# microhh/rte-rrtmgp-cpp

Measured on AMD Instinct MI355X. Metric: columns/sec (LW+SW full solve, 140 lay x 256 gpt), higher is better.
Workload: dtype f64; 1 GPU; C4 synthetic 16384 columns/GPU (16384 in total) x 140 layers x 256 g-points, LW+SW clear-sky, RCEMIP profile, synthetic k-distribution (real shapes); columns_per_gpu=16384, columns_total=16384, nlay=140, ngpt=256, flux_mode=broadband (do_broadband solvers, g-point sums on chip), columns_sorted=False, parallelism=columns sharded x1, all-gather of broadband fluxes

## Files before the change

### include/rrx_hip.h

```cpp
#ifndef RRX_HIP_H
#define RRX_HIP_H

#ifdef __cplusplus
extern "C" {
#endif

typedef signed char RrxBool;

const char* rrx_last_error(void);
int rrx_device_count(int* n);
int rrx_set_device(int dev);
int rrx_malloc(void** ptr, unsigned long long bytes);
int rrx_free(void* ptr);
int rrx_malloc_async(void** ptr, unsigned long long bytes, void* stream);
int rrx_free_async(void* ptr, void* stream);
int rrx_free_async_ordered(void* ptr, void* alloc_stream, void* release_stream);
int rrx_memcpy_h2d_stream(void* dst, const void* src, unsigned long long bytes, void* stream);
int rrx_memcpy_d2h_stream(void* dst, const void* src, unsigned long long bytes, void* stream);
int rrx_memcpy_h2d(void* dst, const void* src, unsigned long long bytes);
int rrx_memcpy_d2h(void* dst, const void* src, unsigned long long bytes);
int rrx_memcpy_d2d(void* dst, const void* src, unsigned long long bytes, void* stream);
int rrx_memset(void* dst, int value, unsigned long long bytes, void* stream);
int rrx_synchronize(void* stream);
int rrx_stream_create(void** stream);
int rrx_stream_destroy(void* stream);
int rrx_release_workspace(void* stream);
int rrx_identity_columns(int ncol, int npad, int* perm, void* stream);
unsigned long long rrx_workspace_bytes(void* stream);
int rrx_subset_nd(void* out, const void* in, int elem_bytes, int ndim, const int* sub_dims, const long long* strides,
                  const int* starts, const int* spread, void* stream);
int rrx_set_lw_variant(int v);
int rrx_set_sw_variant(int v);
int rrx_set_broadband_min_groups(int n);
int rrx_set_broadband_gsplit(int n);
int rrx_set_gas_window(int on);
int rrx_gas_window_stats(long long* handed_back, long long* workgroups, int reset);

#define RRX_DECLARE(F, SFX) \
 \
 \
int rrx_apply_BC_factor##SFX(int ncol, int nlay, int ngpt, RrxBool top_at_1, const F* inc_flux_dir, const F* mu0, F* gpt_flux_dir, void* stream); \
int rrx_apply_BC_0##SFX(int ncol, int nlay, int ngpt, RrxBool top_at_1, F* gpt_flux_dn, void* stream); \
int rrx_apply_BC_gpt##SFX(int ncol, int nlay, int ngpt, RrxBool top_at_1, const F* inc_flux_dif, F* gpt_flux_dn, void* stream); \
 \
int rrx_lw_secants_array##SFX(int ncol, int ngpt, int n_gauss_quad, int max_gauss_pts, const F* gauss_Ds, F* secants, void* stream); \
 \
int rrx_lw_solver_noscat##SFX( \
        int ncol, int nlay, int ngpt, RrxBool top_at_1, int nmus, \
        const F* secants, const F* weights, \
        const F* tau, const F* lay_source, const F* lev_source, \
        const F* sfc_emis, const F* sfc_src, const F* inc_flux, \
// ... 306 lines not shown
```

### rte-rrtmgp-cpp_amd/csrc/rrx_gas_optics.hip

```cpp
#include <type_traits>
#include <cstdio>
#include <cstdlib>
#include "rrx_common.h"
#include "rrx_hip.h"

namespace
{
#ifndef RRX_GW_NT
#define RRX_GW_NT 1
#endif
#ifndef RRX_GW_ABL
#define RRX_GW_ABL 0
#endif
template<typename F> __device__ __forceinline__ void stream_store_sbase(const char* sbase, const unsigned voff, const F v)
{
    static_assert(sizeof(F) == 4 || sizeof(F) == 8, "dword or dwordx2");
    if (RRX_GW_ABL == 7) { if (v == F(-12345.678)) *reinterpret_cast<F*>(const_cast<char*>(sbase) + voff) = v; return; }
#if RRX_GW_NT
    if constexpr (sizeof(F) == 4) asm volatile("global_store_dword %0, %1, %2 nt" :: "v"(voff), "v"(v), "s"(sbase) : "memory");
    else asm volatile("global_store_dwordx2 %0, %1, %2 nt" :: "v"(voff), "v"(v), "s"(sbase) : "memory");
#else
    if constexpr (sizeof(F) == 4) asm volatile("global_store_dword %0, %1, %2" :: "v"(voff), "v"(v), "s"(sbase) : "memory");
    else asm volatile("global_store_dwordx2 %0, %1, %2" :: "v"(voff), "v"(v), "s"(sbase) : "memory");
#endif
// ... 1220 lines not shown
template<typename F> struct PlanckArgs
{
    const F* pfracin; const F* tlev; const F* tsfc; int sfc_lay; int nPlanckTemp; const int* gpoint_bands;
    F totplnk_delta; const F* totplnk; F* pfrac; F* blay; F* blev; F* sfc_src; F* sfc_src_jac;
};

struct GasWindowTables
{
    int ngpt, nmax, ncmax;
    static constexpr int LIT = 1 + NXW;
    __host__ __device__ int off_cinfo() const { return 2*ngpt; }
    __host__ __device__ int off_lists() const { return off_cinfo() + ncmax + 3; }
    __host__ __device__ int off_mmeta() const { return off_lists() + 2*ncmax*LIT; }
    __host__ __device__ int off_cuni()  const { return off_mmeta() + 2*MM*nmax; }
    __host__ __device__ int off_order() const { return off_cuni() + 2*ncmax; }
    __host__ __device__ int ints()      const { return (off_order() + 2*ncmax + 3) & ~3; }
};
inline int gas_window_ncmax(const int ngpt, const int nband) { return (ngpt + GCH - 1) / GCH + std::max(nband, 0); }

constexpr int GW_TBL_HEADER = 8;
constexpr int GW_TBL_MAGIC = 0x52525834;
__global__ void __launch_bounds__(256)
gas_window_tables_kernel(
        const int ngpt, const int nminorlower, const int nminorupper, const int ncmax, const int nlist,
        const int* __restrict__ gpoint_flavor,
        const int* __restrict__ minor_limits_gpt_lower, const int* __restrict__ minor_limits_gpt_upper,
        const Bool* __restrict__ minor_scales_with_density_lower, const Bool* __restrict__ minor_scales_with_density_upper,
        const Bool* __restrict__ scale_by_complement_lower, const Bool* __restrict__ scale_by_complement_upper,
        const int* __restrict__ idx_minor_lower, const int* __restrict__ idx_minor_upper,
        const int* __restrict__ idx_minor_scaling_lower, const int* __restrict__ idx_minor_scaling_upper,
        const int* __restrict__ kminor_start_lower, const int* __restrict__ kminor_start_upper,
        int* __restrict__ tbl)
{
    extern __shared__ int lds_int[];
    const int nmax = max(nminorlower, nminorupper);
    const GasWindowTables T{ngpt, nmax, ncmax};
    constexpr int LIT = GasWindowTables::LIT;
    int* gflav = lds_int;
    int* cinfo = lds_int + T.off_cinfo();
    int* lists = lds_int + T.off_lists();
    int* mmeta = lds_int + T.off_mmeta();
    int* cuni = lds_int + T.off_cuni();
    int* order = lds_int + T.off_order();
    int* cut = lds_int + T.ints();
    const int tid = threadIdx.x;
    const int ntab = T.ints();
    for (int w = tid; w < ntab + ngpt + 4 + 2*((ngpt + 63)/64); w += 256) lds_int[w] = 0;
    __syncthreads();
    {
        for (int w = tid; w < 2*ngpt; w += 256) gflav[(w & 1)*ngpt + (w >> 1)] = gpoint_flavor[w] - 1;
        for (int w = tid; w < nminorlower; w += 256)
        {
            int* m = mmeta + MM*w;
            m[0] = idx_minor_lower[w]; m[1] = minor_scales_with_density_lower[w] ? 1 : 0;
            m[2] = idx_minor_scaling_lower[w]; m[3] = scale_by_complement_lower[w] ? 1 : 0;
            m[4] = minor_limits_gpt_lower[2*w]; m[5] = minor_limits_gpt_lower[2*w+1]; m[6] = kminor_start_lower[w];
        }
        for (int w = tid; w < nminorupper; w += 256)
        {
            int* m = mmeta + MM*(nmax + w);
            m[0] = idx_minor_upper[w]; m[1] = minor_scales_with_density_upper[w] ? 1 : 0;
            m[2] = idx_minor_scaling_upper[w]; m[3] = scale_by_complement_upper[w] ? 1 : 0;
            m[4] = minor_limits_gpt_upper[2*w]; m[5] = minor_limits_gpt_upper[2*w+1]; m[6] = kminor_start_upper[w];
        }
    }
    __syncthreads();
    {
        int* head = tbl + ntab;
        int differs = (head[0] != GW_TBL_MAGIC || head[1] != ngpt || head[2] != nminorlower || head[3] != nminorupper
                       || head[4] != ncmax || head[5] != nlist) ? 1 : 0;
        for (int w = tid; w < 2*ngpt && !differs; w += 256) differs = (tbl[w] != gflav[w]) ? 1 : 0;
        for (int w = tid; w < 2*MM*nmax && !differs; w += 256) differs = (tbl[T.off_mmeta() + w] != mmeta[w]) ? 1 : 0;
        if (!__syncthreads_or(differs)) return;
        if (tid == 0) head[0] = 0;
    }
    for (int g = tid; g < ngpt; g += 256)
        if (g > 0 && (gflav[g] != gflav[g-1] || gflav[ngpt + g] != gflav[ngpt + g-1])) cut[g] = 1;
    for (int w = tid; w < 2*nmax; w += 256)
    {
        const int r = w / nmax, i = w % nmax;
        if (i < (r == 0 ? nminorlower : nminorupper))
        {
            const int* m = mmeta + MM*w;
            const int lo = m[4]-1, hi = m[5];
            if (lo > 0 && lo < ngpt) cut[lo] = 1;
            if (hi > 0 && hi < ngpt) cut[hi] = 1;
        }
// ... 74 lines not shown
            for (int d=c; d<nchunk; ++d) if (gflav[tid*ngpt + cinfo[2 + d]] == fl) ord[k++] = d;
        }
    }

    __syncthreads();
#ifdef RRX_GW_DEBUG_TABLES
    if (tid == 0)
    {
        printf("tables: ngpt %d ncmax %d chunks %d regular %d\n", ngpt, ncmax, cinfo[0], cinfo[1]);
        for (int c=0; c<nchunk; ++c)
            printf("  chunk %d [%d,%d) lower: n %d usable %d fl %d | upper: n %d usable %d fl %d\n", c, cinfo[2+c], cinfo[3+c],
                   lists[c*LIT], cuni[c], gflav[cinfo[2+c]], lists[(ncmax + c)*LIT], cuni[ncmax + c], gflav[ngpt + cinfo[2+c]]);
    }
#endif
    for (int w = tid; w < ntab; w += 256) tbl[w] = lds_int[w];
    __threadfence();
    __syncthreads();
    if (tid == 0)
    {
        int* head = tbl + ntab;
        head[1] = ngpt; head[2] = nminorlower; head[3] = nminorupper; head[4] = ncmax; head[5] = nlist;
        __threadfence();
        head[0] = GW_TBL_MAGIC;
    }
}

inline int* gas_window_tables(hipStream_t st, const int* key_ptr, const int ngpt, const int nminorlower, const int nminorupper,
                              const int ncmax, const int nlist)
{
    struct Entry { int dev; const int* key; int dims[5]; int* buf; };
    static thread_local std::vector<Entry> cache;
    int dev = 0;
    if (hipGetDevice(&dev) != hipSuccess) throw std::runtime_error("no device");
    const int dims[5] = {ngpt, nminorlower, nminorupper, ncmax, nlist};
    for (const Entry& e : cache)
        if (e.dev == dev && e.key == key_ptr && std::equal(dims, dims + 5, e.dims)) return e.buf;
    (void)st;
    if (cache.size() >= 32) { (void)hipFree(cache.front().buf); cache.erase(cache.begin()); }
    const size_t n = size_t(GasWindowTables{ngpt, std::max(nminorlower, nminorupper), ncmax}.ints()) + GW_TBL_HEADER;
    Entry e{dev, key_ptr, {dims[0], dims[1], dims[2], dims[3], dims[4]}, nullptr};
    if (hipMalloc(reinterpret_cast<void**>(&e.buf), n*sizeof(int)) != hipSuccess) throw std::runtime_error("table allocation failed");
    if (hipMemset(e.buf, 0, n*sizeof(int)) != hipSuccess) throw std::runtime_error("memset failed");
    cache.push_back(e);
    return e.buf;
}

template<typename F>
size_t gas_window_lds_bytes(const int ngpt, const int nmax, const int ncmax, const int mode, const bool pf)
{
    const size_t ints = size_t(GasWindowTables{ngpt, nmax, ncmax}.ints()) + 16 + 8*size_t(ncmax);
    const size_t pairs = size_t(GCH)*WBOX*(pf ? 2 : 1) + size_t(NCW)*GCH*MBOX + (mode == 1 ? size_t(GCH)*MBOX : 0);
    return ((ints*sizeof(int) + 15) & ~size_t(15)) + pairs*2*sizeof(F);
}

#ifndef RRX_GW_MINW
#define RRX_GW_MINW 3
#endif
template<typename F, int MODE, bool PF, bool CLD = false>
__global__ void __launch_bounds__(256, RRX_GW_MINW)
gas_window_kernel(
        const int ncol, const int nlay, const int ngpt, const int neta, const int npres, const int ntemp,
        const int nminorlower, const int nminorupper, const int idx_h2o,
        const int* __restrict__ gpoint_flavor,
        const F* __restrict__ kmajor, const F* __restrict__ kminor_lower, const F* __restrict__ kminor_upper,
        const int* __restrict__ minor_limits_gpt_lower, const int* __restrict__ minor_limits_gpt_upper,
// ... 2 lines not shown
        const int* __restrict__ idx_minor_lower, const int* __restrict__ idx_minor_upper,
        const int* __restrict__ idx_minor_scaling_lower, const int* __restrict__ idx_minor_scaling_upper,
        const int* __restrict__ kminor_start_lower, const int* __restrict__ kminor_start_upper,
        const F* __restrict__ play, const F* __restrict__ tlay, const F* __restrict__ col_gas, const F* __restrict__ col_dry,
        const F* __restrict__ krayl, const InterpArgs<F> ia,
        F* __restrict__ tau, F* __restrict__ ssa, F* __restrict__ g, const PlanckArgs<F> pa,
        int* __restrict__ todo, const int geom, const int* __restrict__ tbl, const int ncmax)
{
    #pragma clang fp contract(fast)
    typedef F Vec2 __attribute__((ext_vector_type(2)));
    typedef F Vec2u __attribute__((ext_vector_type(2), aligned(sizeof(F))));
    (void)sizeof(Vec2u);
    extern __shared__ int lds_int[];
    const int nmax = max(nminorlower, nminorupper);
    const GasWindowTables T{ngpt, nmax, ncmax};
    constexpr int LIT = GasWindowTables::LIT;
    int* gflav = lds_int;
    const int* cinfo = lds_int + T.off_cinfo();
    const int* cstart = cinfo + 2;
    int* lists = lds_int + T.off_lists();
    int* mmeta = lds_int + T.off_mmeta();
    int* cuni = lds_int + T.off_cuni();
    int* red = lds_int + T.ints();
    int* cband = red + 16;
    const size_t int_bytes = ((size_t(T.ints()) + 16 + 8*size_t(ncmax))*sizeof(int) + 15) & ~size_t(15);
    Vec2* Wmaj = reinterpret_cast<Vec2*>(reinterpret_cast<char*>(lds_int) + int_bytes);
    Vec2* Wpf  = Wmaj + GCH*WBOX;
    Vec2* Wmin = Wpf + (PF ? GCH*WBOX : 0);
    Vec2* Wray = Wmin + NCW*GCH*MBOX;

    const int tid = threadIdx.y*64 + threadIdx.x;
#if RRX_GW_TIMING
    unsigned long long gw_acc[8] = {0, 0, 0, 0, 0, 0, 0, 0}, gw_t = __builtin_readcyclecounter();
#endif
    {
        const int n4 = T.ints() / 4;
        const int4* __restrict__ src = reinterpret_cast<const int4*>(tbl);
        int4* dst = reinterpret_cast<int4*>(lds_int);
        for (int w = tid; w < n4; w += 256) dst[w] = src[w];
        if (tid < 16) red[tid] = (tid >= 6) ? 0 : ((tid & 1) ? -2147483647 : 2147483647);
    }

    const int icol_raw = geom ? (blockIdx.x*4 + threadIdx.y)*64 + threadIdx.x : blockIdx.x*64 + threadIdx.x;
    const int ilay_raw = geom ? int(blockIdx.y) : blockIdx.y*4 + threadIdx.y;
    const bool active = icol_raw < ncol && ilay_raw < nlay;
    const int icol = min(icol_raw, ncol-1), ilay = min(ilay_raw, nlay-1);
    const size_t ncl = size_t(ncol)*nlay;
    const size_t idx = icol + size_t(ilay)*ncol;
    const F pl = play[idx], tl = tlay[idx];
    const CellState<F> cs = cell_state<F>(ia, npres, ntemp, pl, tl);
    const int itr = cs.itropo;
    const int jt = cs.jt, jp = cs.jp_raw + itr;

    __syncthreads();
    atomicMin(&red[0], jt); atomicMax(&red[1], jt); atomicMin(&red[2], jp); atomicMax(&red[3], jp);
    atomicMin(&red[4], itr); atomicMax(&red[5], itr);
    if (tid < cinfo[0])
    {
        const int c0_ = cstart[tid], ge_ = cstart[tid+1];
        if constexpr (PF) { cband[8*tid] = pa.gpoint_bands[c0_] - 1; cband[8*tid+1] = pa.gpoint_bands[ge_-1] - 1; }
        if constexpr (CLD)
        {
            int b0 = 0;
            while (c0_ + 1 > ia.cld_lims[2*b0+1]) ++b0;
            cband[8*tid+2] = b0; cband[8*tid+3] = (ge_ <= ia.cld_lims[2*b0+1]) ? 1 : 0;
        }
        #pragma unroll
        for (int r=0; r<2; ++r)
        {
            const int fl_ = gflav[r*ngpt + c0_];
            cband[8*tid+4+2*r] = ia.flavor[2*fl_]; cband[8*tid+5+2*r] = ia.flavor[2*fl_+1];
        }
    }
    __syncthreads();
    const int jt_lo = red[0], jp_lo = red[2];
    const int nchunk = rfl(cinfo[0]);
    const bool whole_range = gridDim.z > 1 && rfl(cinfo[1]) == 0;
    if (whole_range && blockIdx.z > 0) return;
    const int c_per = whole_range ? nchunk : (nchunk + int(gridDim.z) - 1) / int(gridDim.z);
    const int c_lo = whole_range ? 0 : int(blockIdx.z)*c_per, c_hi = min(nchunk, c_lo + c_per);
    bool fits = (red[1] - jt_lo < NTW) && (red[3] - jp_lo + 2 <= NPW) && (red[4] == red[5]);
    {
        bool all_chunks = true;
        for (int c=c_lo; c<c_hi; ++c) all_chunks = all_chunks && (cuni[itr*ncmax + c] != 0);
        fits = fits && all_chunks;
    }
    auto hand_back = [&](const int why)
    {
        if (tid == 0)
        {
            const int k = atomicAdd(&todo[0], 1);
            todo[1 + k] = int(blockIdx.y*gridDim.x + blockIdx.x) + int(whole_range ? gridDim.z : blockIdx.z)*int(gridDim.x*gridDim.y);
            atomicAdd(&todo[why - 8], 1);
        }
    };
    if (!fits)
    {
        hand_back(!(red[1] - jt_lo < NTW) ? 0 : !(red[3] - jp_lo + 2 <= NPW) ? 1 : (red[4] != red[5]) ? 2 : 3);
        return;
    }
// ... 1 lines not shown
    const int tn = ntemp*neta;
    const size_t s_gpt = size_t(ntemp)*neta*(npres+1);
    constexpr unsigned SZ = sizeof(F);
    const F cdry0 = col_gas[idx];
    const F ch2o = col_gas[idx + size_t(idx_h2o)*ncl];
    F ray_fac = F(0.);
    if constexpr (MODE == 1) ray_fac = ch2o + col_dry[idx];
    const int ti = jt - jt_lo;
    const int pi0 = jp - jp_lo;

    const unsigned idx_b = unsigned(idx)*SZ;
    auto slab_store = [&](F* __restrict__ arr, const int ig, const F v)
    {
        stream_store(reinterpret_cast<F*>(reinterpret_cast<char*>(arr + size_t(ig)*ncl) + idx_b), v);
    };
    auto minor_scaling = [&](const int imnr) -> F
    {
        const int* m = mmeta + MM*(itr*nmax + imnr);
        const int imn = rfl(m[0]), swd = rfl(m[1]), ims = rfl(m[2]), sbc = rfl(m[3]);
        F scaling = col_gas[idx + size_t(imn)*ncl];
        const F cscal = col_gas[idx + size_t(max(ims, 0))*ncl];
        if (swd)
        {
            scaling *= F(0.01) * pl / tl;
            if (ims > 0)
            {
                const F vmr_fact = F(1.) / cdry0;
                const F dry_fact = F(1.) / (F(1.) + ch2o * vmr_fact);
                const F x = cscal * vmr_fact * dry_fact;
                scaling *= sbc ? (F(1.) - x) : x;
            }
        }
        return scaling;
    };

    [[maybe_unused]] F b_sfc = F(0.), b_sfc2 = F(0.);
    [[maybe_unused]] bool is_last = false, is_sfc = false;
    [[maybe_unused]] int cur_bnd = -1;
    [[maybe_unused]] const size_t ncv = size_t(ncol)*(nlay+1);
    [[maybe_unused]] F t_lev = F(0.);
    if constexpr (PF)
    {
        is_last = ilay == nlay-1; is_sfc = ilay == pa.sfc_lay-1;
        t_lev = pa.tlev[idx];
    }
    if constexpr (PF)
    {
        const int b_first = rfl(cband[8*c_lo]), b_last = rfl(cband[8*(c_hi-1)+1]);
        const size_t ncv_ = size_t(ncol)*(nlay+1);
        const Interp1dPos<F> p_lay = interp1d_pos(tl, ia.temp_ref_min, pa.totplnk_delta, pa.nPlanckTemp);
        const Interp1dPos<F> p_lev = interp1d_pos(t_lev, ia.temp_ref_min, pa.totplnk_delta, pa.nPlanckTemp);
        Interp1dPos<F> p_levp = p_lev;
        if (is_last) p_levp = interp1d_pos(pa.tlev[idx + ncol], ia.temp_ref_min, pa.totplnk_delta, pa.nPlanckTemp);
        #pragma unroll 4
        for (int ib=b_first; ib<=b_last; ++ib)
        {
            const F* tp = pa.totplnk + size_t(ib)*pa.nPlanckTemp;
            const F bl = interp1d_at(p_lay, tp), bv = interp1d_at(p_lev, tp);
            if (active) { pa.blay[idx + size_t(ib)*ncl] = bl; pa.blev[idx + size_t(ib)*ncv_] = bv; }
            if (is_last && active) pa.blev[idx + ncol + size_t(ib)*ncv_] = interp1d_at(p_levp, tp);
        }
    }


    int cur_flav = -1, je_lo = 1;
    [[maybe_unused]] int ne_x = NEW;
    [[maybe_unused]] int cb = 0, cb_have = -1;
    [[maybe_unused]] F c_tau = F(0.), c_ssa = F(0.), c_g = F(0.);
    F fm[8], cm[2], fn[4]; int je[2] = {1, 1};
    #pragma unroll
    for (int i=0; i<8; ++i) fm[i] = F(0.);
    cm[0] = cm[1] = F(0.); fn[0] = fn[1] = fn[2] = fn[3] = F(0.);
    const F* kmin = itr == 0 ? kminor_lower : kminor_upper;
    int red_slot = 6;

    if (RRX_GW_ABL == 1) return;
    RRX_GW_T(0)
    const int* corder = lds_int + T.off_order() + rfl(itr)*ncmax;
    auto item_meta = [&](const int* items, const int i, int& lo, int& hi, int& koff)
    {
        const int* m = mmeta + MM*(rfl(itr)*nmax + rfl(items[i]));
        lo = rfl(m[4]) - 1; hi = rfl(m[5]); koff = rfl(m[6]) - 1 - lo;
    };
    for (int kc=c_lo; kc<c_hi; ++kc)
    {
        const int c = (gridDim.z == 1 || whole_range) ? rfl(corder[kc]) : kc;
        const int c0 = rfl(cstart[c]), gend = rfl(cstart[c+1]), ng = gend - c0;
        const int fl = gflav[itr*ngpt + c0];
        if (fl != cur_flav)
        {
            cur_flav = fl;
            const int gas1 = rfl(cband[8*c+4+2*rfl(itr)]), gas2 = rfl(cband[8*c+5+2*rfl(itr)]);
            const F cg1 = col_gas[idx + size_t(gas1)*ncl], cg2 = col_gas[idx + size_t(gas2)*ncl];
            #pragma unroll
            for (int itemp=0; itemp<2; ++itemp)
            {
                F fmi[2], fma[4];
                flavor_state<F>(ia, cs, neta, itemp, gas1, gas2, cg1, cg2, cm[itemp], je[itemp], fmi, fma);
                fn[2*itemp] = fmi[0]; fn[2*itemp+1] = fmi[1];
                fm[4*itemp] = fma[0]; fm[4*itemp+1] = fma[1]; fm[4*itemp+2] = fma[2]; fm[4*itemp+3] = fma[3];
            }
            unsigned present = 0u;
            for (int j=1; j<neta; ++j)
                if (__ballot(je[0] == j || je[1] == j) != 0ull) present |= (1u << j);
            if (threadIdx.x == 0) atomicOr(reinterpret_cast<unsigned*>(&red[red_slot]), present);
            __syncthreads();
            const unsigned all_present = reinterpret_cast<unsigned*>(red)[red_slot];
            je_lo = __ffs(int(all_present)) - 1;
            const int je_hi = 31 - __clz(int(all_present));
            red_slot = (red_slot == 6) ? 8 : 6;
            if (tid == 0) red[red_slot] = 0;
            if (je_hi - je_lo + 2 > NEW) { hand_back(4); return; }
            ne_x = je_hi - je_lo + 2;
        }
        const int itr_s = rfl(itr);
        const int n_all = rfl(lists[(itr_s*ncmax + c)*LIT]);
        const int n = min(n_all, NCW);
        const int* items = lists + (itr_s*ncmax + c)*LIT + 1;

        [[maybe_unused]] auto cld_arrived = [&]()
        {
            if constexpr (CLD)
            {
                if constexpr (MODE != 2) asm volatile("" : "+v"(c_tau), "+v"(c_ssa), "+v"(c_g));
                else asm volatile("" : "+v"(c_tau));
            }
        };
        [[maybe_unused]] auto cld_load = [&](const int ib)
        {
            if constexpr (CLD)
            {
                cb_have = ib;
                const size_t b = idx + size_t(ib)*ncl;
                c_tau = ia.cld_tau[b];
                if constexpr (MODE != 2) { c_ssa = ia.cld_ssa[b]; c_g = ia.cld_g[b]; }
            }
        };
        [[maybe_unused]] bool cld_one_band = false;
        if constexpr (CLD)
        {
            const int b0 = rfl(cband[8*c+2]);
            cb = b0;
            cld_one_band = rfl(cband[8*c+3]) != 0;
            if (cld_one_band && b0 != cb_have) cld_load(b0);
        }

        RRX_GW_T(1)
        __syncthreads();
        RRX_GW_T(4)
        F sc[NCW]; int slo[NCW], shi[NCW], skoff[NCW];
        auto chunk_scalings = [&]()
        {
            #pragma unroll
            for (int i=0; i<NCW; ++i)
            {
                sc[i] = F(0.); slo[i] = 0; shi[i] = 0; skoff[i] = 0;
                if (i < n) { sc[i] = minor_scaling(rfl(items[i])); item_meta(items, i, slo[i], shi[i], skoff[i]); }
            }
        };
        if (RRX_GW_ABL != 2)
        {
            static_assert((GCH*WBOX) % 256 == 0 && GCH*MBOX <= 256 && NCW == 6, "staging phases are written for these box sizes");
            constexpr int KMAJ = GCH*WBOX/256;
            const int nmaj = ng*WBOX, nmin = ng*MBOX;
            constexpr bool DMA = RRX_GW_LDSDMA && sizeof(F) == 8;
            if constexpr (!DMA || PF) chunk_scalings();
            if constexpr (RRX_GW_SPARSE && (PF || !DMA))
            {
                auto magic = [](const int d) -> unsigned { return 0xFFFFFFFFu / unsigned(d) + 1u; };
                auto divs = [](const int x, const int d, const unsigned m) -> int { return d == 1 ? x : int(__umulhi(unsigned(x), m)); };
                const int np_x = rfl(red[3]) - jp_lo + 2, nt_x = rfl(red[1]) - jt_lo + 1;
                const int et = ne_x*nt_x, wb = np_x*et;
// ... 64 lines not shown
                const int it_ = min(jt_lo - 1 + t, ntemp-2), ie = min(max(je_lo - 1 + e, 0), neta-1), ip = min(max(jp_lo - 1 + p, 0), npres);
                const unsigned off = (unsigned(c0 + gi)*unsigned(s_gpt) + unsigned(it_ + ie*ntemp + ip*tn))*SZ;
                glds(byte_off(kmajor, off), Wmaj + q);
                if constexpr (PF) glds(byte_off(pa.pfracin, off), Wpf + q);
            }
            if (tid < GCH*MBOX)
            {
                const int gi_m = min(tid / MBOX, ng-1), r_m = tid % MBOX;
                const int it_m = min(jt_lo - 1 + r_m % NTW, ntemp-2), ie_m = min(max(je_lo - 1 + r_m / NTW, 0), neta-1);
                if constexpr (MODE == 1)
                    glds(byte_off(krayl + size_t(rfl(itr))*tn*ngpt, unsigned((c0 + gi_m)*tn + it_m + ie_m*ntemp)*SZ), Wray + tid);
                #pragma unroll
                for (int i=0; i<NCW; ++i)
                    if (i < n)
                    {
                        int lo, hi, koff; item_meta(items, i, lo, hi, koff);
                        const int kg = min(max(c0 + gi_m, lo), hi-1);
                        glds(byte_off(kmin_u, unsigned((kg + koff)*tn + it_m + ie_m*ntemp)*SZ), Wmin + i*GCH*MBOX + tid);
                    }
            }
            chunk_scalings();
            RRX_GW_T(2)
            asm volatile("s_waitcnt vmcnt(0)" ::: "memory");
            RRX_GW_T(3)
            }
            else
            {
            auto stage_major = [&](const F* __restrict__ table, Vec2* __restrict__ W)
            {
                Vec2 v[KMAJ];
                #pragma unroll
                for (int k=0; k<KMAJ; ++k)
                {
// ... 19 lines not shown
                for (int q = tid; q < nmaj; q += 256)
                {
                    const int gi = q / WBOX, r = q % WBOX;
                    const int p = r / (NEW*NTW), e = (r / NTW) % NEW, t = r % NTW;
                    const int it_ = min(jt_lo - 1 + t, ntemp-2), ie = min(max(je_lo - 1 + e, 0), neta-1), ip = min(max(jp_lo - 1 + p, 0), npres);
                    const size_t off = size_t(c0 + gi)*s_gpt + size_t(it_) + size_t(ie)*ntemp + size_t(ip)*tn;
                    Wmaj[q] = *reinterpret_cast<const Vec2u*>(kmajor + off);
                    Wpf[q] = *reinterpret_cast<const Vec2u*>(pa.pfracin + off);
                }
            }
            __builtin_amdgcn_sched_barrier(0);
            const int gi_m = tid / MBOX, r_m = tid % MBOX;
            const int it_m = min(jt_lo - 1 + r_m % NTW, ntemp-2), ie_m = min(max(je_lo - 1 + r_m / NTW, 0), neta-1);
            auto minor_node = [&](const int i) -> Vec2
            {
                int lo, hi, koff; item_meta(items, i, lo, hi, koff);
                const int kg = min(max(c0 + gi_m, lo), hi-1);
                return *reinterpret_cast<const Vec2u*>(kmin + size_t(kg + koff)*tn + it_m + ie_m*ntemp);
            };
            if (tid < nmin)
            {
                Vec2 v[3]; [[maybe_unused]] Vec2 vray;
                if constexpr (MODE == 1)
                    vray = *reinterpret_cast<const Vec2u*>(krayl + size_t(itr)*tn*ngpt + size_t(c0 + gi_m)*tn + it_m + ie_m*ntemp);
                #pragma unroll
                for (int i=0; i<3; ++i) if (i < n) v[i] = minor_node(i);
                if constexpr (MODE == 1) Wray[tid] = vray;
                #pragma unroll
                for (int i=0; i<3; ++i) if (i < n) Wmin[(i*GCH + gi_m)*MBOX + r_m] = v[i];
                if (n > 3)
                {
                    #pragma unroll
                    for (int i=3; i<NCW; ++i) if (i < n) v[i-3] = minor_node(i);
// ... 20 lines not shown
            {
                cur_bnd = ibnd;
                const F* tp = pa.totplnk + size_t(ibnd)*pa.nPlanckTemp;
                if (is_sfc)
                {
                    const F t_sfc = pa.tsfc[icol];
                    b_sfc  = interp1d(t_sfc        , ia.temp_ref_min, pa.totplnk_delta, pa.nPlanckTemp, tp);
                    b_sfc2 = interp1d(t_sfc + F(1.), ia.temp_ref_min, pa.totplnk_delta, pa.nPlanckTemp, tp);
                }
            }
        };
        if constexpr (CLD) cld_arrived();
        [[maybe_unused]] bool one_band = false;
        if constexpr (PF)
        {
            const int b0 = rfl(cband[8*c]), b1 = rfl(cband[8*c+1]);
            one_band = b0 == b1;
            if (one_band && b0 != cur_bnd) band_update(b0);
        }
        RRX_GW_T(1)

        unsigned cmask[NCW];
        #pragma unroll
        for (int i=0; i<NCW; ++i)
        {
            const int lo = max(slo[i] - c0, 0), hi = min(shi[i] - c0, ng);
            cmask[i] = (i < n && hi > lo) ? (((hi >= 32) ? ~0u : ((1u << hi) - 1u)) & ~((1u << lo) - 1u)) : 0u;
        }
        const size_t slab_b = ncl*SZ;
        char* sb_tau = reinterpret_cast<char*>(tau) + size_t(c0)*slab_b;
        [[maybe_unused]] char* sb_ssa = (MODE != 2) ? reinterpret_cast<char*>(ssa) + size_t(c0)*slab_b : nullptr;
// ... 179 lines not shown
                if (wave_same_eta) gloop(T_{}, F_{}); else gloop(F_{}, F_{});
            }
            if constexpr (MODE != 2 && !CLD)
            {
                if (g != nullptr && active)
                    for (int gi=0; gi<ng; ++gi) slab_store(g, c0 + gi, F(0.));
            }
        }
        if constexpr (MODE == 2)
        if (n_all > NCW)
        {
            const F* kmin_u = rfl(itr) == 0 ? kminor_lower : kminor_upper;
            for (int x=NCW; x<n_all; ++x)
            {
                __syncthreads();
                int xlo, xhi, xk; item_meta(items, x, xlo, xhi, xk);
                if (tid < GCH*MBOX)
                {
                    const int gi_m = min(tid / MBOX, ng-1), r_m = tid % MBOX;
                    const int it_m = min(jt_lo - 1 + r_m % NTW, ntemp-2), ie_m = min(max(je_lo - 1 + r_m / NTW, 0), neta-1);
                    const int kg = min(max(c0 + gi_m, xlo), xhi-1);
                    Wmin[tid] = *reinterpret_cast<const Vec2u*>(kmin_u + size_t(kg + xk)*tn + it_m + ie_m*ntemp);
                }
                const F scx = minor_scaling(rfl(items[x]));
                __syncthreads();
                asm volatile("s_waitcnt vmcnt(0)" ::: "memory");
                for (int gi=0; gi<ng; ++gi)
                {
                    const int ig = c0 + gi;
                    if (ig < xlo || ig >= xhi) continue;
                    const Vec2* wn = Wmin + gi*MBOX;
                    const Vec2 c0v = wn[q0], c1v = wn[q0 + NTW];
                    F m2 = c0v.y, m3 = c1v.y;
                    if (!wave_same_eta) { m2 = wn[q1].y; m3 = wn[q1 + NTW].y; }
                    const F add = (fn[0]*c0v.x + fn[1]*c1v.x + fn[2]*m2 + fn[3]*m3) * scx;
                    F* tp = reinterpret_cast<F*>(reinterpret_cast<char*>(tau + size_t(ig)*ncl) + idx_b);
                    if (active)
                    {
                        const F tt = __hip_atomic_load(tp, __ATOMIC_RELAXED, __HIP_MEMORY_SCOPE_AGENT) + add;
// ... 71 lines not shown
    const int ncmax = gas_window_ncmax(ngpt, nband);
    const size_t wlds = gas_window_lds_bytes<F>(ngpt, nmax, ncmax, 2, true);
    const bool windowed = tuning().go_window && wlds <= 64*1024 && size_t(ncol)*nlay*sizeof(F) < (size_t(1) << 32)
                          && size_t(ngpt)*ntemp*neta*(npres+1)*sizeof(F) < (size_t(1) << 32);
    StreamScratch scratch(st);
    const int geom = gas_window_geometry(ncol);
    const dim3 wgrid = gas_window_grid(geom, ncol, nlay);
    const int nblk = windowed ? int(wgrid.x)*int(wgrid.y) : int(grid.x)*int(grid.y);
    const int nz = gas_window_parts(nblk, nchunk);
    int* todo = nullptr;
    if (windowed)
    {
        todo = scratch.get<int>(size_t(9) + size_t(nblk)*nz) + 8;
        if (hipMemsetAsync(todo - 8, 0, 9*sizeof(int), st) != hipSuccess) throw std::runtime_error("memset failed");
        const GasWindowTables T{ngpt, nmax, ncmax};
        int* tbl = gas_window_tables(st, gpoint_flavor, ngpt, nminorlower, nminorupper, ncmax, NXW);
        gas_window_tables_kernel<<<1, 256, size_t(T.ints() + ngpt + 4 + 2*((ngpt + 63)/64))*sizeof(int), st>>>(
                ngpt, nminorlower, nminorupper, ncmax, NXW, gpoint_flavor, minor_limits_gpt_lower, minor_limits_gpt_upper,
                minor_scales_with_density_lower, minor_scales_with_density_upper, scale_by_complement_lower, scale_by_complement_upper,
                idx_minor_lower, idx_minor_upper, idx_minor_scaling_lower, idx_minor_scaling_upper,
                kminor_start_lower, kminor_start_upper, tbl);
        const PlanckArgs<F> pa{pfracin, tlev, tsfc, sfc_lay, nPlanckTemp, gpoint_bands, totplnk_delta, totplnk, pfrac, blay, blev, sfc_src, sfc_src_jac};
#define RRX_GW_PF_ARGS ncol, nlay, ngpt, neta, npres, ntemp, nminorlower, nminorupper, idx_h2o, gpoint_flavor, \
                kmajor, kminor_lower, kminor_upper, minor_limits_gpt_lower, minor_limits_gpt_upper, \
                minor_scales_with_density_lower, minor_scales_with_density_upper, \
                scale_by_complement_lower, scale_by_complement_upper, \
                idx_minor_lower, idx_minor_upper, idx_minor_scaling_lower, idx_minor_scaling_upper, \
                kminor_start_lower, kminor_start_upper, play, tlay, col_gas, (const F*)nullptr, (const F*)nullptr, ia, \
                tau, (F*)nullptr, (F*)nullptr, pa, todo, geom, tbl, ncmax
        if (ia.cld_tau != nullptr) gas_window_kernel<F,2,true,true><<<dim3(wgrid.x, wgrid.y, nz), block, wlds, st>>>(RRX_GW_PF_ARGS);
        else gas_window_kernel<F,2,true><<<dim3(wgrid.x, wgrid.y, nz), block, wlds, st>>>(RRX_GW_PF_ARGS);
#undef RRX_GW_PF_ARGS
        gas_window_stats("lw + fractions", todo, nblk*nz, st);
// ... 47 lines not shown
    {
        const int ncmax = gas_window_ncmax(ngpt, nband);
        const size_t wlds = gas_window_lds_bytes<F>(ngpt, nmax, ncmax, MODE, false);
        if (tuning().go_window && wlds <= 64*1024 && size_t(ncol)*nlay*sizeof(F) < (size_t(1) << 32)
            && size_t(ngpt)*ntemp*neta*(npres+1)*sizeof(F) < (size_t(1) << 32))
        {
            hipStream_t st = static_cast<hipStream_t>(stream);
            StreamScratch scratch(st);
            const int geom = gas_window_geometry(ncol);
            const dim3 wgrid = gas_window_grid(geom, ncol, nlay);
            const int nblk = int(wgrid.x)*int(wgrid.y);
            const int nz = gas_window_parts(nblk, nchunk);
            int* todo = scratch.get<int>(size_t(9) + size_t(nblk)*nz) + 8;
            if (hipMemsetAsync(todo - 8, 0, 9*sizeof(int), st) != hipSuccess) throw std::runtime_error("memset failed");
            const GasWindowTables T{ngpt, nmax, ncmax};
            int* tbl = gas_window_tables(st, gpoint_flavor, ngpt, nminorlower, nminorupper, ncmax, (MODE == 1) ? NCW : NXW);
            gas_window_tables_kernel<<<1, 256, size_t(T.ints() + ngpt + 4 + 2*((ngpt + 63)/64))*sizeof(int), st>>>(
                    ngpt, nminorlower, nminorupper, ncmax, (MODE == 1) ? NCW : NXW, gpoint_flavor, minor_limits_gpt_lower, minor_limits_gpt_upper,
                    minor_scales_with_density_lower, minor_scales_with_density_upper, scale_by_complement_lower, scale_by_complement_upper,
                    idx_minor_lower, idx_minor_upper, idx_minor_scaling_lower, idx_minor_scaling_upper,
                    kminor_start_lower, kminor_start_upper, tbl);
#define RRX_GW_ARGS ncol, nlay, ngpt, neta, npres, ntemp, nminorlower, nminorupper, idx_h2o, gpoint_flavor, \
                    kmajor, kminor_lower, kminor_upper, minor_limits_gpt_lower, minor_limits_gpt_upper, \
                    minor_scales_with_density_lower, minor_scales_with_density_upper, \
                    scale_by_complement_lower, scale_by_complement_upper, \
                    idx_minor_lower, idx_minor_upper, idx_minor_scaling_lower, idx_minor_scaling_upper, \
                    kminor_start_lower, kminor_start_upper, play, tlay, col_gas, col_dry, krayl, ia, tau, ssa, g, \
                    PlanckArgs<F>(), todo, geom, tbl, ncmax
#define RRX_TA_ARGS ncol, nlay, ngpt, neta, npres, ntemp, nminorlower, nminorupper, idx_h2o, gpoint_flavor, \
                    kmajor, kminor_lower, kminor_upper, minor_limits_gpt_lower, minor_limits_gpt_upper, \
                    minor_scales_with_density_lower, minor_scales_with_density_upper, \
                    scale_by_complement_lower, scale_by_complement_upper, \
                    idx_minor_lower, idx_minor_upper, idx_minor_scaling_lower, idx_minor_scaling_upper, \
// ... 370 lines not shown
    reorder12x21_kernel<F><<<grid1d(size_t(ni)*nj), 256, 0, static_cast<hipStream_t>(stream)>>>(ni, nj, arr_in, arr_out); \
    RRX_CATCH("rrx_reorder12x21") \
} \
int rrx_zero_array##SFX(int ni, int nj, int nk, F* arr, void* stream) \
{ \
    RRX_TRY \
    if (hipMemsetAsync(arr, 0, size_t(ni)*nj*nk*sizeof(F), static_cast<hipStream_t>(stream)) != hipSuccess) \
        throw std::runtime_error("hipMemsetAsync failed"); \
    RRX_CATCH("rrx_zero_array") \
}

RRX_DEFINE_GAS(double, _f64)
RRX_DEFINE_GAS(float, _f32)
}

extern "C" int rrx_gas_window_stats(long long* handed_back, long long* workgroups, int reset)
{
    if (handed_back) *handed_back = g_gw_handed;
    if (workgroups) *workgroups = g_gw_total;
    if (reset) { g_gw_handed = 0; g_gw_total = 0; }
    return 0;
}
```

Measured before the change: 1.425 million columns/s.

## Read gas-window chunk metadata from precomputed constant-memory records instead of LDS copies

The table-building kernel now also precomputes per-chunk records (chunk bounds, flavor, gases, bands, cloud band, order, minor-item descriptors) plus a prefix count of non-uniform chunks. The windowed gas-optics kernel reads these records through scalar/constant address-space vector loads instead of copying the whole table into LDS and recomputing band and flavor info per workgroup. This cuts LDS footprint and per-workgroup setup, which could raise occupancy. It also makes table allocation stream-ordered with an event, and adds a debug readback API.

```diff
diff --git a/include/rrx_hip.h b/include/rrx_hip.h
--- a/include/rrx_hip.h
+++ b/include/rrx_hip.h
@@ -35,6 +35,7 @@
 int rrx_set_broadband_gsplit(int n);
 int rrx_set_gas_window(int on);
 int rrx_gas_window_stats(long long* handed_back, long long* workgroups, int reset);
+int rrx_gas_window_tables_read(int* tables, int capacity, int* layout);
 
 #define RRX_DECLARE(F, SFX) \
  \
diff --git a/rte-rrtmgp-cpp_amd/csrc/rrx_gas_optics.hip b/rte-rrtmgp-cpp_amd/csrc/rrx_gas_optics.hip
--- a/rte-rrtmgp-cpp_amd/csrc/rrx_gas_optics.hip
+++ b/rte-rrtmgp-cpp_amd/csrc/rrx_gas_optics.hip
@@ -1258,16 +1258,25 @@
     __host__ __device__ int off_mmeta() const { return off_lists() + 2*ncmax*LIT; }
     __host__ __device__ int off_cuni()  const { return off_mmeta() + 2*MM*nmax; }
     __host__ __device__ int off_order() const { return off_cuni() + 2*ncmax; }
-    __host__ __device__ int ints()      const { return (off_order() + 2*ncmax + 3) & ~3; }
+    static constexpr int GX = 6;
+    static constexpr int RH = 12;
+    static constexpr int RC = 8;
+    static constexpr int REC = RH + RC*NXW;
+    __host__ __device__ int off_gx()    const { return (off_order() + 2*ncmax + 3) & ~3; }
+    __host__ __device__ int off_bad()   const { return off_gx() + GX*ngpt; }
+    __host__ __device__ int off_rec()   const { return (off_bad() + 2*(ncmax + 1) + 3) & ~3; }
+    __host__ __device__ int ints()      const { return off_rec() + 2*ncmax*REC; }
 };
+static_assert(GasWindowTables::REC % 4 == 0 && GasWindowTables::RH % 4 == 0 && GasWindowTables::RC == 8, "records are read as 16- and 32-byte words");
 inline int gas_window_ncmax(const int ngpt, const int nband) { return (ngpt + GCH - 1) / GCH + std::max(nband, 0); }
 
 constexpr int GW_TBL_HEADER = 8;
-constexpr int GW_TBL_MAGIC = 0x52525834;
+constexpr int GW_TBL_MAGIC = 0x52525835;
 __global__ void __launch_bounds__(256)
 gas_window_tables_kernel(
-        const int ngpt, const int nminorlower, const int nminorupper, const int ncmax, const int nlist,
+        const int ngpt, const int nminorlower, const int nminorupper, const int ncmax, const int nlist, const int nband,
         const int* __restrict__ gpoint_flavor,
+        const int* __restrict__ flavor, const int* __restrict__ gpoint_bands, const int* __restrict__ band_lims,
         const int* __restrict__ minor_limits_gpt_lower, const int* __restrict__ minor_limits_gpt_upper,
         const Bool* __restrict__ minor_scales_with_density_lower, const Bool* __restrict__ minor_scales_with_density_upper,
         const Bool* __restrict__ scale_by_complement_lower, const Bool* __restrict__ scale_by_complement_upper,
@@ -1286,9 +1295,21 @@
     int* mmeta = lds_int + T.off_mmeta();
     int* cuni = lds_int + T.off_cuni();
     int* order = lds_int + T.off_order();
-    int* cut = lds_int + T.ints();
+    int* cut = lds_int + T.off_gx();
     const int tid = threadIdx.x;
-    const int ntab = T.ints();
+    const int ntab = T.off_gx();
+    auto gx_of = [&](const int g, const int k) -> int
+    {
+        if (k == 0) return gpoint_bands != nullptr ? gpoint_bands[g] - 1 : -1;
+        if (k == 1)
+        {
+            if (band_lims == nullptr) return -1;
+            int b = 0;
+            while (b < nband-1 && g + 1 > band_lims[2*b+1]) ++b;
+            return b;
+        }
+        return flavor[2*gflav[((k - 2) >> 1)*ngpt + g] + (k & 1)];
+    };
     for (int w = tid; w < ntab + ngpt + 4 + 2*((ngpt + 63)/64); w += 256) lds_int[w] = 0;
     __syncthreads();
     {
@@ -1310,11 +1331,13 @@
     }
     __syncthreads();
     {
-        int* head = tbl + ntab;
+        int* head = tbl + T.ints();
         int differs = (head[0] != GW_TBL_MAGIC || head[1] != ngpt || head[2] != nminorlower || head[3] != nminorupper
-                       || head[4] != ncmax || head[5] != nlist) ? 1 : 0;
+                       || head[4] != ncmax || head[5] != nlist || head[6] != nband) ? 1 : 0;
         for (int w = tid; w < 2*ngpt && !differs; w += 256) differs = (tbl[w] != gflav[w]) ? 1 : 0;
         for (int w = tid; w < 2*MM*nmax && !differs; w += 256) differs = (tbl[T.off_mmeta() + w] != mmeta[w]) ? 1 : 0;
+        for (int w = tid; w < GasWindowTables::GX*ngpt && !differs; w += 256)
+            differs = (tbl[T.off_gx() + w] != gx_of(w / GasWindowTables::GX, w % GasWindowTables::GX)) ? 1 : 0;
         if (!__syncthreads_or(differs)) return;
         if (tid == 0) head[0] = 0;
     }
@@ -1419,41 +1442,87 @@
     }
 #endif
     for (int w = tid; w < ntab; w += 256) tbl[w] = lds_int[w];
+    for (int w = tid; w < GasWindowTables::GX*ngpt; w += 256) tbl[T.off_gx() + w] = gx_of(w / GasWindowTables::GX, w % GasWindowTables::GX);
+    if (tid < 2)
+    {
+        int* bad = tbl + T.off_bad() + tid*(ncmax + 1);
+        int k = 0;
+        for (int c=0; c<=ncmax; ++c) { bad[c] = k; if (c < nchunk && cuni[tid*ncmax + c] == 0) ++k; }
+    }
+    for (int w = tid; w < 2*ncmax; w += 256)
+    {
+        constexpr int RH = GasWindowTables::RH, RC = GasWindowTables::RC, REC = GasWindowTables::REC;
+        const int r = w / ncmax, c = w % ncmax;
+        int* rec = tbl + T.off_rec() + w*REC;
+        for (int k=0; k<REC; ++k) rec[k] = 0;
+        if (c >= nchunk) continue;
+        const int c0 = cinfo[2 + c], c1 = cinfo[3 + c];
+        const int* li = lists + w*LIT;
+        rec[0] = c0; rec[1] = c1; rec[2] = gflav[r*ngpt + c0]; rec[3] = li[0];
+        rec[4] = gx_of(c0, 2 + 2*r); rec[5] = gx_of(c0, 3 + 2*r);
+        rec[6] = gx_of(c0, 0); rec[7] = gx_of(c1 - 1, 0);
+        const int b0 = gx_of(c0, 1);
+        rec[8] = b0; rec[9] = (b0 >= 0 && c1 <= band_lims[2*b0+1]) ? 1 : 0;
+        rec[10] = cuni[w]; rec[11] = order[w];
+        for (int i=0; i<min(li[0], nlist); ++i)
+        {
+            const int* m = mmeta + MM*(r*nmax + li[1 + i]);
+            int* o = rec + RH + RC*i;
+            const int lo = m[4] - 1;
+            o[0] = lo; o[1] = m[5]; o[2] = m[6] - 1 - lo; o[3] = m[0]; o[4] = m[1]; o[5] = m[2]; o[6] = m[3];
+        }
+    }
     __threadfence();
     __syncthreads();
     if (tid == 0)
     {
-        int* head = tbl + ntab;
-        head[1] = ngpt; head[2] = nminorlower; head[3] = nminorupper; head[4] = ncmax; head[5] = nlist;
+        int* head = tbl + T.ints();
+        head[1] = ngpt; head[2] = nminorlower; head[3] = nminorupper; head[4] = ncmax; head[5] = nlist; head[6] = nband;
         __threadfence();
         head[0] = GW_TBL_MAGIC;
     }
 }
 
+struct GasWindowLast { int* buf = nullptr; int ngpt = 0, nmax = 0, ncmax = 0; };
+thread_local GasWindowLast g_gw_last;
 inline int* gas_window_tables(hipStream_t st, const int* key_ptr, const int ngpt, const int nminorlower, const int nminorupper,
-                              const int ncmax, const int nlist)
-{
-    struct Entry { int dev; const int* key; int dims[5]; int* buf; };
+                              const int ncmax, const int nlist, const int extras)
+{
+    struct Entry { int dev; const int* key; int dims[6]; int* buf; hipStream_t made_on; hipEvent_t zeroed; };
     static thread_local std::vector<Entry> cache;
     int dev = 0;
     if (hipGetDevice(&dev) != hipSuccess) throw std::runtime_error("no device");
-    const int dims[5] = {ngpt, nminorlower, nminorupper, ncmax, nlist};
+    const int dims[6] = {ngpt, nminorlower, nminorupper, ncmax, nlist, extras};
+    g_gw_last.ngpt = ngpt; g_gw_last.nmax = std::max(nminorlower, nminorupper); g_gw_last.ncmax = ncmax;
     for (const Entry& e : cache)
-        if (e.dev == dev && e.key == key_ptr && std::equal(dims, dims + 5, e.dims)) return e.buf;
-    (void)st;
-    if (cache.size() >= 32) { (void)hipFree(cache.front().buf); cache.erase(cache.begin()); }
+        if (e.dev == dev && e.key == key_ptr && std::equal(dims, dims + 6, e.dims))
+        {
+            if (e.made_on != st && hipStreamWaitEvent(st, e.zeroed, 0) != hipSuccess) throw std::runtime_error("stream wait failed");
+            g_gw_last.buf = e.buf;
+            return e.buf;
+        }
+    if (cache.size() >= 32)
+    {
+        Entry& old = cache.front();
+        (void)hipStreamWaitEvent(st, old.zeroed, 0); (void)hipFreeAsync(old.buf, st); (void)hipEventDestroy(old.zeroed);
+        cache.erase(cache.begin());
+    }
     const size_t n = size_t(GasWindowTables{ngpt, std::max(nminorlower, nminorupper), ncmax}.ints()) + GW_TBL_HEADER;
-    Entry e{dev, key_ptr, {dims[0], dims[1], dims[2], dims[3], dims[4]}, nullptr};
-    if (hipMalloc(reinterpret_cast<void**>(&e.buf), n*sizeof(int)) != hipSuccess) throw std::runtime_error("table allocation failed");
-    if (hipMemset(e.buf, 0, n*sizeof(int)) != hipSuccess) throw std::runtime_error("memset failed");
+    Entry e{dev, key_ptr, {dims[0], dims[1], dims[2], dims[3], dims[4], dims[5]}, nullptr, st, nullptr};
+    if (hipMallocAsync(reinterpret_cast<void**>(&e.buf), n*sizeof(int), st) != hipSuccess) throw std::runtime_error("table allocation failed");
+    if (hipMemsetAsync(e.buf, 0, n*sizeof(int), st) != hipSuccess) throw std::runtime_error("memset failed");
+    if (hipEventCreateWithFlags(&e.zeroed, hipEventDisableTiming) != hipSuccess || hipEventRecord(e.zeroed, st) != hipSuccess)
+        throw std::runtime_error("event failed");
     cache.push_back(e);
+    g_gw_last.buf = e.buf;
     return e.buf;
 }
 
 template<typename F>
 size_t gas_window_lds_bytes(const int ngpt, const int nmax, const int ncmax, const int mode, const bool pf)
 {
-    const size_t ints = size_t(GasWindowTables{ngpt, nmax, ncmax}.ints()) + 16 + 8*size_t(ncmax);
+    (void)ngpt; (void)nmax; (void)ncmax;
+    const size_t ints = 16;
     const size_t pairs = size_t(GCH)*WBOX*(pf ? 2 : 1) + size_t(NCW)*GCH*MBOX + (mode == 1 ? size_t(GCH)*MBOX : 0);
     return ((ints*sizeof(int) + 15) & ~size_t(15)) + pairs*2*sizeof(F);
 }
@@ -1486,16 +1555,13 @@
     extern __shared__ int lds_int[];
     const int nmax = max(nminorlower, nminorupper);
     const GasWindowTables T{ngpt, nmax, ncmax};
-    constexpr int LIT = GasWindowTables::LIT;
-    int* gflav = lds_int;
-    const int* cinfo = lds_int + T.off_cinfo();
-    const int* cstart = cinfo + 2;
-    int* lists = lds_int + T.off_lists();
-    int* mmeta = lds_int + T.off_mmeta();
-    int* cuni = lds_int + T.off_cuni();
-    int* red = lds_int + T.ints();
-    int* cband = red + 16;
-    const size_t int_bytes = ((size_t(T.ints()) + 16 + 8*size_t(ncmax))*sizeof(int) + 15) & ~size_t(15);
+    typedef int Int4 __attribute__((ext_vector_type(4)));
+    typedef int Int8 __attribute__((ext_vector_type(8)));
+    typedef const __attribute__((address_space(4))) int* CInt;
+    const CInt ctbl = reinterpret_cast<CInt>(reinterpret_cast<uintptr_t>(tbl));
+    constexpr int RH = GasWindowTables::RH, RC = GasWindowTables::RC, REC = GasWindowTables::REC;
+    int* red = lds_int;
+    const size_t int_bytes = 16*sizeof(int);
     Vec2* Wmaj = reinterpret_cast<Vec2*>(reinterpret_cast<char*>(lds_int) + int_bytes);
     Vec2* Wpf  = Wmaj + GCH*WBOX;
     Vec2* Wmin = Wpf + (PF ? GCH*WBOX : 0);
@@ -1506,10 +1572,6 @@
     unsigned long long gw_acc[8] = {0, 0, 0, 0, 0, 0, 0, 0}, gw_t = __builtin_readcyclecounter();
 #endif
     {
-        const int n4 = T.ints() / 4;
-        const int4* __restrict__ src = reinterpret_cast<const int4*>(tbl);
-        int4* dst = reinterpret_cast<int4*>(lds_int);
-        for (int w = tid; w < n4; w += 256) dst[w] = src[w];
         if (tid < 16) red[tid] = (tid >= 6) ? 0 : ((tid & 1) ? -2147483647 : 2147483647);
     }
 
@@ -1527,35 +1589,17 @@
     __syncthreads();
     atomicMin(&red[0], jt); atomicMax(&red[1], jt); atomicMin(&red[2], jp); atomicMax(&red[3], jp);
     atomicMin(&red[4], itr); atomicMax(&red[5], itr);
-    if (tid < cinfo[0])
-    {
-        const int c0_ = cstart[tid], ge_ = cstart[tid+1];
-        if constexpr (PF) { cband[8*tid] = pa.gpoint_bands[c0_] - 1; cband[8*tid+1] = pa.gpoint_bands[ge_-1] - 1; }
-        if constexpr (CLD)
-        {
-            int b0 = 0;
-            while (c0_ + 1 > ia.cld_lims[2*b0+1]) ++b0;
-            cband[8*tid+2] = b0; cband[8*tid+3] = (ge_ <= ia.cld_lims[2*b0+1]) ? 1 : 0;
-        }
-        #pragma unroll
-        for (int r=0; r<2; ++r)
-        {
-            const int fl_ = gflav[r*ngpt + c0_];
-            cband[8*tid+4+2*r] = ia.flavor[2*fl_]; cband[8*tid+5+2*r] = ia.flavor[2*fl_+1];
-        }
-    }
     __syncthreads();
     const int jt_lo = red[0], jp_lo = red[2];
-    const int nchunk = rfl(cinfo[0]);
-    const bool whole_range = gridDim.z > 1 && rfl(cinfo[1]) == 0;
+    const int nchunk = ctbl[T.off_cinfo()];
+    const bool whole_range = gridDim.z > 1 && ctbl[T.off_cinfo() + 1] == 0;
     if (whole_range && blockIdx.z > 0) return;
     const int c_per = whole_range ? nchunk : (nchunk + int(gridDim.z) - 1) / int(gridDim.z);
     const int c_lo = whole_range ? 0 : int(blockIdx.z)*c_per, c_hi = min(nchunk, c_lo + c_per);
     bool fits = (red[1] - jt_lo < NTW) && (red[3] - jp_lo + 2 <= NPW) && (red[4] == red[5]);
     {
-        bool all_chunks = true;
-        for (int c=c_lo; c<c_hi; ++c) all_chunks = all_chunks && (cuni[itr*ncmax + c] != 0);
-        fits = fits && all_chunks;
+        const CInt bad = ctbl + T.off_bad() + rfl(red[4])*(ncmax + 1);
+        fits = fits && (bad[c_hi] == bad[c_lo]);
     }
     auto hand_back = [&](const int why)
     {
@@ -1587,10 +1631,8 @@
     {
         stream_store(reinterpret_cast<F*>(reinterpret_cast<char*>(arr + size_t(ig)*ncl) + idx_b), v);
     };
-    auto minor_scaling = [&](const int imnr) -> F
-    {
-        const int* m = mmeta + MM*(itr*nmax + imnr);
-        const int imn = rfl(m[0]), swd = rfl(m[1]), ims = rfl(m[2]), sbc = rfl(m[3]);
+    auto minor_scaling = [&](const int imn, const int swd, const int ims, const int sbc) -> F
+    {
         F scaling = col_gas[idx + size_t(imn)*ncl];
         const F cscal = col_gas[idx + size_t(max(ims, 0))*ncl];
         if (swd)
@@ -1619,7 +1661,8 @@
     }
     if constexpr (PF)
     {
-        const int b_first = rfl(cband[8*c_lo]), b_last = rfl(cband[8*(c_hi-1)+1]);
+        const CInt rec0 = ctbl + T.off_rec() + rfl(itr)*ncmax*REC;
+        const int b_first = rec0[c_lo*REC + 6], b_last = rec0[(c_hi-1)*REC + 7];
         const size_t ncv_ = size_t(ncol)*(nlay+1);
         const Interp1dPos<F> p_lay = interp1d_pos(tl, ia.temp_ref_min, pa.totplnk_delta, pa.nPlanckTemp);
         const Interp1dPos<F> p_lev = interp1d_pos(t_lev, ia.temp_ref_min, pa.totplnk_delta, pa.nPlanckTemp);
@@ -1649,21 +1692,21 @@
 
     if (RRX_GW_ABL == 1) return;
     RRX_GW_T(0)
-    const int* corder = lds_int + T.off_order() + rfl(itr)*ncmax;
-    auto item_meta = [&](const int* items, const int i, int& lo, int& hi, int& koff)
-    {
-        const int* m = mmeta + MM*(rfl(itr)*nmax + rfl(items[i]));
-        lo = rfl(m[4]) - 1; hi = rfl(m[5]); koff = rfl(m[6]) - 1 - lo;
-    };
+    const CInt recs = ctbl + T.off_rec() + rfl(itr)*ncmax*REC;
     for (int kc=c_lo; kc<c_hi; ++kc)
     {
-        const int c = (gridDim.z == 1 || whole_range) ? rfl(corder[kc]) : kc;
-        const int c0 = rfl(cstart[c]), gend = rfl(cstart[c+1]), ng = gend - c0;
-        const int fl = gflav[itr*ngpt + c0];
+        const int c = (gridDim.z == 1 || whole_range) ? recs[kc*REC + 11] : kc;
+        const CInt rec = recs + c*REC;
+        const Int4 rh0 = *reinterpret_cast<const __attribute__((address_space(4))) Int4*>(rec);
+        const Int4 rh1 = *reinterpret_cast<const __attribute__((address_space(4))) Int4*>(rec + 4);
+        [[maybe_unused]] const Int4 rh2 = *reinterpret_cast<const __attribute__((address_space(4))) Int4*>(rec + 8);
+        auto item_rec = [&](const int i) -> Int8 { return *reinterpret_cast<const __attribute__((address_space(4))) Int8*>(rec + RH + RC*i); };
+        const int c0 = rh0.x, gend = rh0.y, ng = gend - c0;
+        const int fl = rh0.z;
         if (fl != cur_flav)
         {
             cur_flav = fl;
-            const int gas1 = rfl(cband[8*c+4+2*rfl(itr)]), gas2 = rfl(cband[8*c+5+2*rfl(itr)]);
+            const int gas1 = rh1.x, gas2 = rh1.y;
             const F cg1 = col_gas[idx + size_t(gas1)*ncl], cg2 = col_gas[idx + size_t(gas2)*ncl];
             #pragma unroll
             for (int itemp=0; itemp<2; ++itemp)
@@ -1686,10 +1729,8 @@
             if (je_hi - je_lo + 2 > NEW) { hand_back(4); return; }
             ne_x = je_hi - je_lo + 2;
         }
-        const int itr_s = rfl(itr);
-        const int n_all = rfl(lists[(itr_s*ncmax + c)*LIT]);
+        const int n_all = rh0.w;
         const int n = min(n_all, NCW);
-        const int* items = lists + (itr_s*ncmax + c)*LIT + 1;
 
         [[maybe_unused]] auto cld_arrived = [&]()
         {
@@ -1712,9 +1753,9 @@
         [[maybe_unused]] bool cld_one_band = false;
         if constexpr (CLD)
         {
-            const int b0 = rfl(cband[8*c+2]);
+            const int b0 = rh2.x;
             cb = b0;
-            cld_one_band = rfl(cband[8*c+3]) != 0;
+            cld_one_band = rh2.y != 0;
             if (cld_one_band && b0 != cb_have) cld_load(b0);
         }
 
@@ -1728,7 +1769,7 @@
             for (int i=0; i<NCW; ++i)
             {
                 sc[i] = F(0.); slo[i] = 0; shi[i] = 0; skoff[i] = 0;
-                if (i < n) { sc[i] = minor_scaling(rfl(items[i])); item_meta(items, i, slo[i], shi[i], skoff[i]); }
+                if (i < n) { const Int8 m = item_rec(i); sc[i] = minor_scaling(m.s3, m.s4, m.s5, m.s6); slo[i] = m.s0; shi[i] = m.s1; skoff[i] = m.s2; }
             }
         };
         if (RRX_GW_ABL != 2)
@@ -1823,9 +1864,9 @@
                 for (int i=0; i<NCW; ++i)
                     if (i < n)
                     {
-                        int lo, hi, koff; item_meta(items, i, lo, hi, koff);
-                        const int kg = min(max(c0 + gi_m, lo), hi-1);
-                        glds(byte_off(kmin_u, unsigned((kg + koff)*tn + it_m + ie_m*ntemp)*SZ), Wmin + i*GCH*MBOX + tid);
+                        const Int8 m = item_rec(i);
+                        const int kg = min(max(c0 + gi_m, m.s0), m.s1-1);
+                        glds(byte_off(kmin_u, unsigned((kg + m.s2)*tn + it_m + ie_m*ntemp)*SZ), Wmin + i*GCH*MBOX + tid);
                     }
             }
             chunk_scalings();
@@ -1875,9 +1916,9 @@
             const int it_m = min(jt_lo - 1 + r_m % NTW, ntemp-2), ie_m = min(max(je_lo - 1 + r_m / NTW, 0), neta-1);
             auto minor_node = [&](const int i) -> Vec2
             {
-                int lo, hi, koff; item_meta(items, i, lo, hi, koff);
-                const int kg = min(max(c0 + gi_m, lo), hi-1);
-                return *reinterpret_cast<const Vec2u*>(kmin + size_t(kg + koff)*tn + it_m + ie_m*ntemp);
+                const Int8 m = item_rec(i);
+                const int kg = min(max(c0 + gi_m, m.s0), m.s1-1);
+                return *reinterpret_cast<const Vec2u*>(kmin + size_t(kg + m.s2)*tn + it_m + ie_m*ntemp);
             };
             if (tid < nmin)
             {
@@ -1928,7 +1969,7 @@
         [[maybe_unused]] bool one_band = false;
         if constexpr (PF)
         {
-            const int b0 = rfl(cband[8*c]), b1 = rfl(cband[8*c+1]);
+            const int b0 = rh1.z, b1 = rh1.w;
             one_band = b0 == b1;
             if (one_band && b0 != cur_bnd) band_update(b0);
         }
@@ -2138,7 +2179,8 @@
             for (int x=NCW; x<n_all; ++x)
             {
                 __syncthreads();
-                int xlo, xhi, xk; item_meta(items, x, xlo, xhi, xk);
+                const Int8 xm = item_rec(x);
+                const int xlo = xm.s0, xhi = xm.s1, xk = xm.s2;
                 if (tid < GCH*MBOX)
                 {
                     const int gi_m = min(tid / MBOX, ng-1), r_m = tid % MBOX;
@@ -2146,7 +2188,7 @@
                     const int kg = min(max(c0 + gi_m, xlo), xhi-1);
                     Wmin[tid] = *reinterpret_cast<const Vec2u*>(kmin_u + size_t(kg + xk)*tn + it_m + ie_m*ntemp);
                 }
-                const F scx = minor_scaling(rfl(items[x]));
+                const F scx = minor_scaling(xm.s3, xm.s4, xm.s5, xm.s6);
                 __syncthreads();
                 asm volatile("s_waitcnt vmcnt(0)" ::: "memory");
                 for (int gi=0; gi<ng; ++gi)
@@ -2248,9 +2290,10 @@
         todo = scratch.get<int>(size_t(9) + size_t(nblk)*nz) + 8;
         if (hipMemsetAsync(todo - 8, 0, 9*sizeof(int), st) != hipSuccess) throw std::runtime_error("memset failed");
         const GasWindowTables T{ngpt, nmax, ncmax};
-        int* tbl = gas_window_tables(st, gpoint_flavor, ngpt, nminorlower, nminorupper, ncmax, NXW);
-        gas_window_tables_kernel<<<1, 256, size_t(T.ints() + ngpt + 4 + 2*((ngpt + 63)/64))*sizeof(int), st>>>(
-                ngpt, nminorlower, nminorupper, ncmax, NXW, gpoint_flavor, minor_limits_gpt_lower, minor_limits_gpt_upper,
+        const int* lims = ia.cld_tau != nullptr ? ia.cld_lims : nullptr;
+        int* tbl = gas_window_tables(st, gpoint_flavor, ngpt, nminorlower, nminorupper, ncmax, NXW, 1 + (lims != nullptr ? 2 : 0));
+        gas_window_tables_kernel<<<1, 256, size_t(T.off_gx() + ngpt + 4 + 2*((ngpt + 63)/64))*sizeof(int), st>>>(
+                ngpt, nminorlower, nminorupper, ncmax, NXW, nband, gpoint_flavor, ia.flavor, gpoint_bands, lims, minor_limits_gpt_lower, minor_limits_gpt_upper,
                 minor_scales_with_density_lower, minor_scales_with_density_upper, scale_by_complement_lower, scale_by_complement_upper,
                 idx_minor_lower, idx_minor_upper, idx_minor_scaling_lower, idx_minor_scaling_upper,
                 kminor_start_lower, kminor_start_upper, tbl);
@@ -2328,9 +2371,10 @@
             int* todo = scratch.get<int>(size_t(9) + size_t(nblk)*nz) + 8;
             if (hipMemsetAsync(todo - 8, 0, 9*sizeof(int), st) != hipSuccess) throw std::runtime_error("memset failed");
             const GasWindowTables T{ngpt, nmax, ncmax};
-            int* tbl = gas_window_tables(st, gpoint_flavor, ngpt, nminorlower, nminorupper, ncmax, (MODE == 1) ? NCW : NXW);
-            gas_window_tables_kernel<<<1, 256, size_t(T.ints() + ngpt + 4 + 2*((ngpt + 63)/64))*sizeof(int), st>>>(
-                    ngpt, nminorlower, nminorupper, ncmax, (MODE == 1) ? NCW : NXW, gpoint_flavor, minor_limits_gpt_lower, minor_limits_gpt_upper,
+            const int* lims = ia.cld_tau != nullptr ? ia.cld_lims : nullptr;
+            int* tbl = gas_window_tables(st, gpoint_flavor, ngpt, nminorlower, nminorupper, ncmax, (MODE == 1) ? NCW : NXW, lims != nullptr ? 2 : 0);
+            gas_window_tables_kernel<<<1, 256, size_t(T.off_gx() + ngpt + 4 + 2*((ngpt + 63)/64))*sizeof(int), st>>>(
+                    ngpt, nminorlower, nminorupper, ncmax, (MODE == 1) ? NCW : NXW, nband, gpoint_flavor, ia.flavor, (const int*)nullptr, lims, minor_limits_gpt_lower, minor_limits_gpt_upper,
                     minor_scales_with_density_lower, minor_scales_with_density_upper, scale_by_complement_lower, scale_by_complement_upper,
                     idx_minor_lower, idx_minor_upper, idx_minor_scaling_lower, idx_minor_scaling_upper,
                     kminor_start_lower, kminor_start_upper, tbl);
@@ -2731,6 +2775,24 @@
 RRX_DEFINE_GAS(float, _f32)
 }
 
+extern "C" int rrx_gas_window_tables_read(int* tables, const int capacity, int* layout)
+{
+    RRX_TRY
+    const GasWindowLast& L = g_gw_last;
+    if (L.buf == nullptr) throw std::runtime_error("no windowed gas-optics launch on this thread yet");
+    const GasWindowTables T{L.ngpt, L.nmax, L.ncmax};
+    const int lay[16] = {T.ints() + GW_TBL_HEADER, L.ngpt, L.nmax, L.ncmax, T.off_cinfo(), T.off_lists(), T.off_mmeta(), T.off_cuni(), T.off_order(),
+                         T.off_gx(), T.off_bad(), T.off_rec(), GasWindowTables::LIT, MM, GasWindowTables::REC, GasWindowTables::RH};
+    if (layout != nullptr) std::copy(lay, lay + 16, layout);
+    if (tables != nullptr)
+    {
+        if (capacity < lay[0]) throw std::runtime_error("buffer too small for the tables");
+        if (hipDeviceSynchronize() != hipSuccess || hipMemcpy(tables, L.buf, size_t(lay[0])*sizeof(int), hipMemcpyDeviceToHost) != hipSuccess)
+            throw std::runtime_error("copy of the tables failed");
+    }
+    RRX_CATCH("rrx_gas_window_tables_read")
+}
+
 extern "C" int rrx_gas_window_stats(long long* handed_back, long long* workgroups, int reset)
 {
     if (handed_back) *handed_back = g_gw_handed;
```

After: 1.441 million columns/s, median of 6. 1.1% higher.
